# B-R-P/NMSLIB-ZIG

Measured on AMD Instinct MI355X. Metric: queries/sec @ recall@10, 1M x 128-D L2, batch=1024; HBM GB/s vs peak, higher is better.
Workload: dtype f16+f32

## Files before the change

nmslib_zig_amd/csrc/kernels/bf_kernels.hip:

```cpp
#include <cstdio>
#include <type_traits>
#include <vector>
#include <cstdlib>

#include "common_dev.hpp"
#include "kernels.hpp"

namespace gfxknn {

enum BfMode : int { BF_L2 = 0, BF_DOT = 1, BF_COS = 2, BF_L1 = 3, BF_LINF = 4, BF_COSC = 5, BF_L2D = 6 };

struct BfArgs {
    const float* base;
    const float* aux;
    const float* qaux;
    int aux_stride;
    const float* queries;
    u64* cand;
    int* cand_cnt;
    uint32_t* gthr;
    uint32_t* gq;
    int xj, xm;
    int n, ldb, nqt, nsplit, rows_per_split, kprime, cap;
    int kcs;
// ... 1422 lines not shown
                    if (have_pv) {
                        const float m = block_max(QG - 1, pv_ax);
                        mfma3_over(0, 0, true);
                        __builtin_amdgcn_sched_barrier(0);
                        finish_check(m, acc[QG - 1], QG - 1, pv_ax, pv_row0);
                    } else {
                        mfma3(0, 0, true, iv);
                    }
                    __builtin_amdgcn_sched_barrier(0);
#pragma unroll
                    for (int g = 1; g < QG; ++g) mfma3(g, 0, true, iv);
                } else if (kc == 7) {
                    mfma3(0, 7, false, acc[0]);
#pragma unroll
                    for (int g = 1; g < QG; ++g) {
                        __builtin_amdgcn_sched_barrier(0);
                        const float m = block_max(g - 1, axs + blk * 32);
                        mfma3_over(g, 7, false);
                        __builtin_amdgcn_sched_barrier(0);
                        finish_check(m, acc[g - 1], g - 1, axs + blk * 32, row0 + blk * 32);
                        __builtin_amdgcn_sched_barrier(0);
                    }
                } else {
#pragma unroll
                    for (int g = 0; g < QG; ++g) mfma3(g, kc, false, acc[0]);
                }
                __builtin_amdgcn_sched_barrier(0);
            }
            pv_ax = axs + blk * 32;
            pv_row0 = row0 + blk * 32;
            have_pv = true;
            if (blk == 0) {
                if (t + 2 < nstages) asm volatile("s_waitcnt vmcnt(9)\n\ts_barrier" ::: "memory");
                else asm volatile("s_waitcnt vmcnt(0)\n\ts_barrier" ::: "memory");
                if (t + kRing - 1 < nstages) issue_tile(t + kRing - 1);
            }
        }
    }
    asm volatile("s_waitcnt lgkmcnt(0)" ::: "memory");
    if (have_pv) finish_check(block_max(QG - 1, pv_ax), acc[QG - 1], QG - 1, pv_ax, pv_row0);
#pragma unroll
    for (int g = 0; g < QG; ++g) {
        const int qidx = (qt * NW + wave) * (32 * QG) + g * 32 + l31;
        if constexpr (SAMPLE) {
            float* o = a.top8 + (((size_t)qidx * a.nsplit + split) * 2 + h) * 8;
#pragma unroll
            for (int i = 0; i < 8; ++i) o[i] = t8[g][i];
        } else {
            a.list_cnt[((size_t)qidx * a.nsplit + split) * 2 + h] = cnt[g];
        }
    }
}

template <int MODE, bool SAMPLE, int QG, int NW, int KCH = 1>
__global__ __launch_bounds__(NW * 64) void bf_scan_bf16_kernel(BfScanF32Args a) {
    extern __shared__ __attribute__((aligned(16))) char smem[];
    const int tid = threadIdx.x, lane = tid & 63, wave = tid >> 6;
    const int h = lane >> 5, l31 = lane & 31;
    const int b = blockIdx.x;
    const int xcd = b & 7, rest = b >> 3;
    const int qt = rest % a.nqt;
    const int split = (rest / a.nqt) * 8 + xcd;
    if (split >= a.nsplit) return;
    if (a.group_flag && (a.group_flag[qt] != 0) != (a.group_want != 0)) return;

    constexpr int kSync = 4, kRing = 2 * kSync + 1, kAuxRing = 16, kStageBytes = BF_BN * 256;
    char* ring = smem;
    float* auxr = reinterpret_cast<float*>(ring + kRing * kStageBytes);
    const int tstr = SAMPLE ? a.tile_stride : 1;
    const int tiles_all = (a.n + BF_BN - 1) / BF_BN;
    const int stiles_all = (tiles_all + tstr - 1) / tstr;
    const int ntiles = max(0, min(a.tps, stiles_all - split * a.tps));
    const int nstages = ntiles * KCH;
    constexpr int kDp = 128 * KCH;
    const int r_begin = split * a.tps * tstr * BF_BN;
    const int stage_rows = tstr * BF_BN;

    uint32_t dma_voff[16 / NW];
#pragma unroll
    for (int jj = 0; jj < 16 / NW; ++jj) {
        const int pj = (16 / NW) * wave + jj;
        const int row = 4 * pj + (lane >> 4);
        const int c = (lane & 15) ^ (row & 15);
        dma_voff[jj] = (uint32_t)((row * kDp + c * 8) * 2);
    }
    const uint32_t dma_lds0 = (uint32_t)(uintptr_t)(lptr_t)ring + (uint32_t)((16 / NW) * __builtin_amdgcn_readfirstlane(wave) * 1024);
    const uint32_t aux_lds0 = (uint32_t)(uintptr_t)(lptr_t)auxr;
    const uint32_t aux_voff = (uint32_t)lane * 4u;
    auto issue_tile = [&](int stage) __attribute__((always_inline)) {
        const int slot = stage % kRing;
        const int row0 = r_begin + (stage / KCH) * stage_rows;
        const unsigned long long sbase = (unsigned long long)(uintptr_t)a.base_h16 + ((unsigned long long)row0 * kDp + (stage % KCH) * 128) * 2ull;
        const uint32_t m0v = dma_lds0 + (uint32_t)slot * kStageBytes;
#pragma clang diagnostic push
#pragma clang diagnostic ignored "-Winline-asm"
#pragma unroll
        for (int jj = 0; jj < 16 / NW; ++jj)
            asm volatile("s_mov_b32 m0, %2\n\ts_nop 0\n\tglobal_load_lds_dwordx4 %0, %1"
                         :: "v"(dma_voff[jj]), "s"(sbase), "s"(m0v + (uint32_t)jj * 1024u) : "memory", "m0");
        const unsigned long long abase = (unsigned long long)(uintptr_t)a.auxp16 + (unsigned long long)row0 * 4ull;
        asm volatile("s_mov_b32 m0, %2\n\ts_nop 0\n\tglobal_load_lds_dword %0, %1"
                     :: "v"(aux_voff), "s"(abase), "s"(aux_lds0 + (uint32_t)((stage % kAuxRing) * BF_BN * 4)) : "memory", "m0");
#pragma clang diagnostic pop
    };

    f16x8 qh[QG][8 * KCH];
    float thr[QG];
    int cnt[QG], ecnt[QG];
    uint32_t* lp[QG];
    float t8[SAMPLE ? QG : 1][8];
#pragma unroll
    for (int g = 0; g < QG; ++g) {
        const int qidx = (qt * NW + wave) * (32 * QG) + g * 32 + l31;
#pragma unroll
        for (int kc = 0; kc < 8 * KCH; ++kc)
            asm volatile("global_load_dwordx4 %0, %1, off" : "=a"(qh[g][kc]) : "v"(static_cast<const _Float16*>(a.q_h16) + (size_t)qidx * kDp + 16 * kc + 8 * h) : "memory");
        cnt[g] = 0;
        ecnt[g] = 0;
        if constexpr (SAMPLE) {
            thr[g] = -INFINITY;
            lp[g] = nullptr;
#pragma unroll
            for (int i = 0; i < 8; ++i) t8[g][i] = -INFINITY;
        } else {
            thr[g] = a.thr[qidx];
            lp[g] = a.list + (size_t)qidx * a.caph * (2 * a.nsplit) + split * 2 + h;
        }
    }
    asm volatile("s_waitcnt vmcnt(0)" ::: "memory");
    for (int t = 0; t <= kSync && t < nstages; ++t) issue_tile(t);
    asm volatile("s_waitcnt vmcnt(0)\n\ts_barrier" ::: "memory");

    uint32_t vad[8];
#pragma unroll
    for (int kc = 0; kc < 8; ++kc)
        vad[kc] = (uint32_t)(uintptr_t)(lptr_t)smem + (uint32_t)(l31 * 256 + (((kc * 2 + h) ^ (l31 & 15)) * 16));

    auto score_of = [&](const f32x16& c, int i, const float* ax) __attribute__((always_inline)) -> float {
        if constexpr (MODE == SC_COS) return c[i] * ax[(i & 3) + 8 * (i >> 2)];
        else return c[i];
    };
    auto block_max_leaves = [&](const f32x16& c, const float* ax, float (&m)[5]) __attribute__((always_inline)) {
#pragma unroll
        for (int j = 0; j < 5; ++j) {
            if constexpr (MODE == SC_COS)
                m[j] = fmaxf(fmaxf(score_of(c, 3 * j, ax), score_of(c, 3 * j + 1, ax)), score_of(c, 3 * j + 2, ax));
            else
                asm("v_max3_f32 %0, %1, %2, %3" : "=v"(m[j]) : "v"(c[3 * j]), "v"(c[3 * j + 1]), "v"(c[3 * j + 2]));
        }
    };
    auto block_max_root = [&](const f32x16& c, const float* ax, const float (&m)[5]) __attribute__((always_inline)) -> float {
        if constexpr (MODE == SC_COS) {
            return fmaxf(fmaxf(fmaxf(m[0], m[1]), m[2]), fmaxf(fmaxf(m[3], m[4]), score_of(c, 15, ax)));
        } else {
            float r0, r1, r;
            asm("v_max3_f32 %0, %1, %2, %3" : "=v"(r0) : "v"(m[0]), "v"(m[1]), "v"(m[2]));
            asm("v_max3_f32 %0, %1, %2, %3" : "=v"(r1) : "v"(m[3]), "v"(m[4]), "v"(c[15]));
            asm("v_max_f32 %0, %1, %2" : "=v"(r) : "v"(r0), "v"(r1));
            return r;
        }
    };
    auto block_max = [&](const f32x16& c, const float* ax) __attribute__((always_inline)) -> float {
        float m[5];
        block_max_leaves(c, ax, m);
        return block_max_root(c, ax, m);
    };
    auto trigger_of = [&](float m, int g) __attribute__((always_inline)) -> unsigned long long {
        return SAMPLE ? __builtin_amdgcn_ballot_w64(m > thr[g]) : __builtin_amdgcn_ballot_w64(m >= thr[g]);
    };
    auto finish_check = [&](unsigned long long trig, float m, const f32x16& c, int g, const float* ax, int row0) __attribute__((always_inline)) {
        if constexpr (SAMPLE) {
            if (__builtin_expect(trig != 0ull, 0)) {
                float v = (row0 + 32 <= a.n || MODE == SC_L2) ? m : -INFINITY;
#pragma unroll
                for (int j = 0; j < 8; ++j) {
                    const float hi = fmaxf(t8[g][j], v);
                    v = fminf(t8[g][j], v);
                    t8[g][j] = hi;
                }
                thr[g] = t8[g][7];
            }
        } else if (__builtin_expect(trig != 0ull, 0)) {
            uint32_t km;
            if constexpr (MODE == SC_COS) {
                f32x16 sc;
#pragma unroll
                for (int i = 0; i < 16; ++i) sc[i] = score_of(c, i, ax);
                km = hit_mask_f32(sc, thr[g]);
            } else {
                km = hit_mask_f32(c, thr[g]);
            }
            if (row0 + 32 > a.n) {
                int nvalid = a.n - row0;
                asm volatile("" : "+s"(nvalid));
#pragma unroll
                for (int i = 0; i < 16; ++i)
                    if (acc_row(i, h) >= nvalid) km &= ~(0x8000u >> i);
            }
            if (km) {
                if (ecnt[g] < a.caph) lp[g][(size_t)ecnt[g] * (2 * a.nsplit)] = ((uint32_t)(row0 - r_begin) >> 5 << 16) | km;
                ecnt[g]++;
                cnt[g] += __builtin_popcount(km);
            }
        }
    };

    f16x8 fh[4];
    f32x16 iv;
#pragma unroll
    for (int i = 0; i < 16; ++i) iv[i] = 0.f;
    f32x16 acc[2][QG];
#pragma unroll
    for (int g = 0; g < QG; ++g) {
#pragma unroll
        for (int i = 0; i < 16; ++i) {
            acc[0][g][i] = 0.f;
            acc[1][g][i] = -INFINITY;
        }
    }
    const float* pv_ax = auxr;
    int pv_row0 = 0;
    bool have_pv = false;
    float m_pend = 0.f;
    unsigned long long trig_pend = 0ull;
    const uint32_t lds0 = (uint32_t)(uintptr_t)(lptr_t)smem;
    auto load_frag = [&](auto off_tag, int kc) __attribute__((always_inline)) {
        constexpr int OFF = decltype(off_tag)::value;
        const uint32_t ad = vad[kc];
        if constexpr (NW == 4) {
            switch (kc % 4) {
                case 0: BF_FRAG_RD_OFF("v[224:227]", fh[0], ad, OFF); break;
                case 1: BF_FRAG_RD_OFF("v[228:231]", fh[1], ad, OFF); break;
                case 2: BF_FRAG_RD_OFF("v[232:235]", fh[2], ad, OFF); break;
                default: BF_FRAG_RD_OFF("v[236:239]", fh[3], ad, OFF); break;
            }
        } else {
            switch (kc % 4) {
                case 0: BF_FRAG_RD_OFF("v[96:99]", fh[0], ad, OFF); break;
                case 1: BF_FRAG_RD_OFF("v[100:103]", fh[1], ad, OFF); break;
                case 2: BF_FRAG_RD_OFF("v[104:107]", fh[2], ad, OFF); break;
                default: BF_FRAG_RD_OFF("v[108:111]", fh[3], ad, OFF); break;
            }
        }
    };
    using Off0 = std::integral_constant<int, 0>;
    using Off1 = std::integral_constant<int, 32 * 256>;
    auto wait_frag = [&](auto cnt_tag, int kc, bool with_init) __attribute__((always_inline)) {
        constexpr int N = decltype(cnt_tag)::value;
#define BF_W1(STR)                                                                                              \
        if constexpr (NW == 4) {                                                                                \
            switch (kc % 4) {                                                                                   \
                case 0:                                                                                         \
                    if (with_init) asm volatile(STR : "+{v[224:227]}"(fh[0]), "+{v[240:255]}"(iv));             \
                    else asm volatile(STR : "+{v[224:227]}"(fh[0]));                                            \
                    break;                                                                                      \
                case 1: asm volatile(STR : "+{v[228:231]}"(fh[1])); break;                                      \
                case 2: asm volatile(STR : "+{v[232:235]}"(fh[2])); break;                                      \
                default: asm volatile(STR : "+{v[236:239]}"(fh[3])); break;                                     \
            }                                                                                                   \
        } else {                                                                                                \
            switch (kc % 4) {                                                                                   \
                case 0:                                                                                         \
                    if (with_init) asm volatile(STR : "+{v[96:99]}"(fh[0]), "+{v[112:127]}"(iv));               \
                    else asm volatile(STR : "+{v[96:99]}"(fh[0]));                                              \
                    break;                                                                                      \
                case 1: asm volatile(STR : "+{v[100:103]}"(fh[1])); break;                                      \
                case 2: asm volatile(STR : "+{v[104:107]}"(fh[2])); break;                                      \
                default: asm volatile(STR : "+{v[108:111]}"(fh[3])); break;                                     \
            }                                                                                                   \
        }
        if constexpr (N == 0) { BF_W1("s_waitcnt lgkmcnt(0)") }
        else if constexpr (N == 2) { BF_W1("s_waitcnt lgkmcnt(2)") }
        else if constexpr (N == 3) { BF_W1("s_waitcnt lgkmcnt(3)") }
        else if constexpr (N == 6) { BF_W1("s_waitcnt lgkmcnt(6)") }
        else { static_assert(N == 7, "wait count"); BF_W1("s_waitcnt lgkmcnt(7)") }
#undef BF_W1
    };
    auto mfma_step = [&](f32x16& c, const f16x8& q, int kc, bool first_ch) __attribute__((always_inline)) {
        if constexpr (MODE == SC_L2) {
            if (kc == 0 && first_ch) {
                if constexpr (NW == 4)
                    asm("v_mfma_f32_32x32x16_f16 %0, %1, %2, %3" : "=&v"(c) : "{v[224:227]}"(fh[0]), "a"(q), "{v[240:255]}"(iv));
                else
                    asm("v_mfma_f32_32x32x16_f16 %0, %1, %2, %3" : "=&v"(c) : "{v[96:99]}"(fh[0]), "a"(q), "{v[112:127]}"(iv));
                return;
            }
        }
        c = __builtin_amdgcn_mfma_f32_32x32x16_f16(fh[kc % 4], q, (kc == 0 && first_ch) ? iv : c, 0, 0, 0);
    };
    auto load_init = [&](uint32_t ax) __attribute__((always_inline)) {
        if constexpr (MODE == SC_L2) {
            if constexpr (NW == 4)
                asm volatile("ds_read_b128 v[240:243], %1\n\tds_read_b128 v[244:247], %1 offset:32\n\t"
                             "ds_read_b128 v[248:251], %1 offset:64\n\tds_read_b128 v[252:255], %1 offset:96"
                             : "={v[240:255]}"(iv) : "v"(ax) : "memory");
            else
                asm volatile("ds_read_b128 v[112:115], %1\n\tds_read_b128 v[116:119], %1 offset:32\n\t"
                             "ds_read_b128 v[120:123], %1 offset:64\n\tds_read_b128 v[124:127], %1 offset:96"
                             : "={v[112:127]}"(iv) : "v"(ax) : "memory");
        }
    };
    constexpr int kInitReads = MODE == SC_L2 ? 4 : 0;
    const uint32_t aux_a = lds0 + kRing * kStageBytes + 16 * h;
    constexpr int kPre = 3;
    auto main_loop = [&](auto stag_tag) __attribute__((always_inline)) {
    constexpr int kStag = decltype(stag_tag)::value;
    if (kStag != 0 && a.prio_half) __builtin_amdgcn_s_setprio(1);
    load_init(aux_a);
#pragma unroll
    for (int kc = 0; kc < kPre; ++kc) load_frag(Off0{}, kc);
    for (int tt = 0; tt < ntiles; ++tt) {
#pragma unroll
      for (int ch = 0; ch < KCH; ++ch) {
        const int t = tt * KCH + ch;
        constexpr bool kOne = KCH == 1;
        const bool first_ch = kOne || ch == 0, last_ch = kOne || ch == KCH - 1;
        const float* axs = auxr + (t % kAuxRing) * BF_BN + 4 * h;
        const int row0 = r_begin + tt * stage_rows;
#pragma unroll
        for (int blk = 0; blk < 2; ++blk) {
            const bool prev_final = blk == 1 ? last_ch : first_ch;
            const bool init_next = blk == 0 ? first_ch : last_ch;
            const int dslot = ((t + 1) % kRing == 0) ? -(kRing - 1) * kStageBytes : kStageBytes;
            const uint32_t nax = blk == 0 ? aux_a + ((t % kAuxRing) * BF_BN + 32) * 4 : aux_a + (((t + 1) % kAuxRing) * BF_BN) * 4;
#pragma unroll
            for (int kc = 0; kc < 8; ++kc) {
                if (kc + kPre < 8) {
                    if (blk == 0) load_frag(Off0{}, kc + kPre);
                    else load_frag(Off1{}, kc + kPre);
                    wait_frag(std::integral_constant<int, kPre>{}, kc, kc == 0 && MODE == SC_L2 && first_ch);
                } else {
                    if (kc == 6 && init_next) load_init(nax);
                    if (blk == 0) {
                        load_frag(Off1{}, kc + kPre - 8);
                    } else {
                        vad[kc + kPre - 8] += (uint32_t)dslot;
                        load_frag(Off0{}, kc + kPre - 8);
                    }
                    if (kInitReads && init_next && kc >= 6) wait_frag(std::integral_constant<int, kPre + 4>{}, kc, false);
                    else wait_frag(std::integral_constant<int, kPre>{}, kc, false);
                }
                __builtin_amdgcn_sched_barrier(0);
                constexpr int kEvery = 8 / QG;
                const int gc = kc >= kStag ? (kc - kStag) / kEvery : 0;
                const bool chk = prev_final && kc >= kStag && ((kc - kStag) % kEvery) == 0;
                const bool br = prev_final && kc >= kStag && ((kc - kStag) % kEvery) == 1;
                float m = 0.f;
                const bool by_hand = MODE == SC_L2 && kc == 0 && first_ch && chk && QG == 2;
                float m5[5];
                if (chk && !by_hand) m = block_max(acc[blk ^ 1][gc], pv_ax);
                mfma_step(acc[blk][0], qh[0][8 * ch + kc], kc, first_ch);
                if (by_hand) {
                    if constexpr (QG == 2) {
                        __builtin_amdgcn_sched_barrier(0);
                        block_max_leaves(acc[blk ^ 1][gc], pv_ax, m5);
                        __builtin_amdgcn_sched_barrier(0);
                        mfma_step(acc[blk][1], qh[1][8 * ch + kc], kc, first_ch);
                        __builtin_amdgcn_sched_barrier(0);
                        m = block_max_root(acc[blk ^ 1][gc], pv_ax, m5);
                    }
                } else if (br) {
                    __builtin_amdgcn_sched_barrier(0);
                    finish_check(trig_pend, m_pend, acc[blk ^ 1][gc], gc, pv_ax, pv_row0);
                    __builtin_amdgcn_sched_barrier(0);
                } else {
                    __builtin_amdgcn_sched_group_barrier(0x008, 1, 0);
                    __builtin_amdgcn_sched_group_barrier(0x002, 12 / QG, 0);
                }
#pragma unroll
                for (int g = 1; g < QG; ++g) {
                    if (by_hand) break;
                    mfma_step(acc[blk][g], qh[g][8 * ch + kc], kc, first_ch);
                    __builtin_amdgcn_sched_group_barrier(0x008, 1, 0);
                    __builtin_amdgcn_sched_group_barrier(0x002, 12 / QG, 0);
                }
                if (chk) {
                    asm volatile("" : "+v"(m));
                    unsigned long long trig = trigger_of(m, gc);
                    asm volatile("" : "+s"(trig));
                    m_pend = m;
                    trig_pend = trig;
                }
                __builtin_amdgcn_sched_barrier(0);
            }
            if (last_ch) {
                pv_ax = axs + blk * 32;
                pv_row0 = row0 + blk * 32;
                have_pv = true;
            }
            if (blk == 1) {
#pragma unroll
                for (int kc = kPre; kc < 8; ++kc) vad[kc] += (uint32_t)dslot;
            }
            if (blk == 0) {
                if (t % kSync == 0) {
                    asm volatile("s_waitcnt vmcnt(0)\n\ts_barrier" ::: "memory");
                    for (int u = t + kSync + 1; u <= t + 2 * kSync && u < nstages; ++u) issue_tile(u);
                }
            }
        }
      }
    }
    asm volatile("s_waitcnt lgkmcnt(0)" ::: "memory");
    };
    if constexpr (NW == 8) {
        if (__builtin_amdgcn_readfirstlane(wave) >= 4) main_loop(std::integral_constant<int, 2>{});
        else main_loop(std::integral_constant<int, 0>{});
    } else {
        main_loop(std::integral_constant<int, 0>{});
    }
    if (have_pv) {
#pragma unroll
        for (int g = 0; g < QG; ++g) {
            const float m = block_max(acc[1][g], pv_ax);
            finish_check(trigger_of(m, g), m, acc[1][g], g, pv_ax, pv_row0);
        }
    }
#pragma unroll
    for (int g = 0; g < QG; ++g) {
        const int qidx = (qt * NW + wave) * (32 * QG) + g * 32 + l31;
        if constexpr (SAMPLE) {
            float* o = a.top8 + (((size_t)qidx * a.nsplit + split) * 2 + h) * 8;
#pragma unroll
            for (int i = 0; i < 8; ++i) o[i] = t8[g][i];
        } else {
            a.list_cnt[((size_t)qidx * a.nsplit + split) * 2 + h] = cnt[g];
        }
    }
}

__global__ void split_bf16_kernel(const float* src, int rows, int rows_pad, int ld, int dim, __bf16* hi, __bf16* lo,
                                  const float* aux, float aux_pad, float* auxp, int dp, _Float16* h16, float scale,
                                  float* auxp16, float aux16_mul) {
    const size_t total = (size_t)rows_pad * dp;
    for (size_t i = (size_t)blockIdx.x * blockDim.x + threadIdx.x; i < total; i += (size_t)gridDim.x * blockDim.x) {
        const size_t r = i / (size_t)dp;
        const int c = (int)(i - r * dp);
        const float v = (r < (size_t)rows && c < dim) ? src[r * ld + c] : 0.f;
        const __bf16 hh = (__bf16)v;
        if (hi) hi[i] = hh;
        if (lo) lo[i] = (__bf16)(v - (float)hh);
        if (h16) h16[i] = (_Float16)(scale * v);
        if (c == 0 && auxp) auxp[r] = r < (size_t)rows ? (aux ? aux[r] : 0.f) : aux_pad;
        if (c == 0 && auxp16) auxp16[r] = r < (size_t)rows ? (aux ? aux[r] * aux16_mul : 0.f) : aux_pad;
    }
}

__global__ void bf_f32_prep_kernel(const float* raw, int nq, int dim, const float* sel, int qpad, int ld, float* pad_out,
                                   __bf16* hi, __bf16* lo, int* clr0, int n0, int* clr1, int n1, uint32_t* clr2, size_t n2,
                                   int dp, _Float16* h16, float scale) {
    const size_t gtid = (size_t)blockIdx.x * blockDim.x + threadIdx.x, gsz = (size_t)gridDim.x * blockDim.x;
    const size_t total = (size_t)qpad * dp;
    for (size_t i = gtid; i < total; i += gsz) {
        const size_t r = i / (size_t)dp;
        const int c = (int)(i - r * dp);
        float v;
        if (raw) {
            v = (r < (size_t)nq && c < dim) ? raw[r * dim + c] : 0.f;
            if (c < ld) pad_out[r * ld + c] = v;
        } else {
            v = c < dim ? sel[r * ld + c] : 0.f;
        }
        const __bf16 hh = (__bf16)v;
        if (hi) hi[i] = hh;
        if (lo) lo[i] = (__bf16)(v - (float)hh);
        h16[i] = (_Float16)(scale * v);
    }
    for (size_t i = gtid; i < (size_t)n0; i += gsz) clr0[i] = 0;
// ... 135 lines not shown
        int run = incl - sum;
        for (int i = 0; i < per; ++i) {
            const int s = tid * per + i;
            if (s < nl) {
                offs[s] = run;
                const int c = a.list_cnt[(size_t)q * nl + s];
                run += c < a.caph ? c : a.caph;
            }
        }
        if (tid == 63) offs[nl] = incl;
        if (__any(over != 0) && tid == 0) s_over = 1;
    } else if (wave == 1) {
        const bool split_product = a.precise[q / a.fail_queries] != 0;
        const float* qs = a.queries_sel + (size_t)q * a.sel_ld;
        float ss = 0.f;
        for (int d = lane; d < a.sel_dim; d += 64) ss = fmaf(qs[d], qs[d], ss);
        ss = wave_sum(ss);
        const float e1 = split_product ? 0.f : one_product_error(qs, a.sel_dim, lane, a.scale * (a.space == SP_L2 || a.space == SP_NEGDOT || a.qaux ? a.bmax : 1.0f), a.bres16, a.scale_q);
        if (lane == 0) {
            s_qn2 = ss;
            s_e1 = e1;
            s_split = split_product ? 1 : 0;
            s_thr = split_product ? a.thr[q] : a.thr1[q];
        }
    }
    __syncthreads();
    const int total = offs[nl];
    if ((a.no_split && a.precise[q / a.fail_queries] != 0) ||
        (a.qaux && a.qaux[(size_t)q * 4 + 3] == 0.f)) {
        if (tid == 0) atomicOr(&a.tile_fail[q / a.fail_queries], 1);
        return;
    }
    const int need = a.k < a.n ? a.k : a.n;
    const int want = need + (a.k / 8 > 4 ? a.k / 8 : 4) < a.n ? need + (a.k / 8 > 4 ? a.k / 8 : 4) : a.n;
    if (s_over || total < want || total > a.p2max) {
        if (tid == 0) atomicOr(&a.tile_fail[q / a.fail_queries], 1);
        return;
    }
    lap(0);
    scan_gather_entries(keys, offs, a.list, q, nl, a.caph, a.tps, tid, blockDim.x);
    __syncthreads();
    lap(1);
    const int P = next_pow2(total < 2 ? 2 : total);
    if (a.prof && tid == 0) {
        atomicAdd(&a.prof[8], (unsigned long long)total);
        atomicAdd(&a.prof[9], (unsigned long long)P);
        atomicAdd(&a.prof[10], 1ull);
    }
    const float* qq = a.queries + (size_t)q * a.ldb;
    const int sub = lane & 15, rg = lane >> 4;
    if (a.dim <= 128) {
        float qv[8];
        bool ok[8];
    #pragma unroll
        for (int c = 0; c < 8; ++c) {
            const int d = sub + 16 * c;
            ok[c] = d < a.dim;
            qv[c] = ok[c] ? qq[d] : 0.f;
        }
        constexpr int kU = 4;
        for (int j0 = wave * (4 * kU); j0 < total; j0 += 16 * kU) {
            uint32_t pos[kU];
            float xv[kU][8];
    #pragma unroll
            for (int u = 0; u < kU; ++u) {
                const int j = j0 + 4 * u + rg;
                pos[u] = (uint32_t)keys[j < total ? j : total - 1];
                const float* row = a.base + (size_t)pos[u] * a.ldb + sub;
    #pragma unroll
                for (int c = 0; c < 8; ++c) xv[u][c] = ok[c] ? row[16 * c] : 0.f;
            }
            __builtin_amdgcn_wave_barrier();
    #pragma unroll
            for (int u = 0; u < kU; ++u) {
                float p0[4], p1[4], p2[4];
    #pragma unroll
                for (int v = 0; v < 4; ++v) {
                    p0[v] = p1[v] = p2[v] = 0.f;
    #pragma unroll
                    for (int c = 0; c < 2; ++c) {
                        if (64 * c >= a.dim) continue;
                        const float x = xv[u][v + 4 * c], y = qv[v + 4 * c];
                        if (a.space == SP_L2) {
                            const float t = x - y;
                            p0[v] = fmaf(t, t, p0[v]);
                        } else {
                            p0[v] = fmaf(x, y, p0[v]);
                            if (a.space != SP_NEGDOT) {
                                p1[v] = fmaf(x, x, p1[v]);
                                p2[v] = fmaf(y, y, p2[v]);
                            }
                        }
                    }
                }
                auto tree = [&](const float* p) __attribute__((always_inline)) -> float {
                    float s = (p[0] + p[2]) + (p[1] + p[3]);
    #pragma unroll
                    for (int o = 8; o > 0; o >>= 1) s += __shfl_xor(s, o, 64);
                    return s;
                };
                const float s0 = tree(p0);
                float d;
                if (a.space == SP_L2) d = sqrtf(s0);
                else if (a.space == SP_NEGDOT) d = -s0;
                else {
                    const float sim = normdot_finish(s0, tree(p1), tree(p2));
                    d = a.space == SP_ANGULAR ? acosf(sim) : fmaxf(0.0f, 1.0f - sim);
                }
                const int j = j0 + 4 * u + rg;
                if (sub == 0 && j < total) keys[j] = ((u64)f32_ord(d) << 32) | pos[u];
            }
        }
    } else {
        const int nstep = (a.dim + 63) >> 6;
        for (int j0 = wave * 16; j0 < total; j0 += 64) {
            uint32_t pos[4];
            const float* rowp[4];
    #pragma unroll
            for (int u = 0; u < 4; ++u) {
                const int j = j0 + 4 * u + rg;
                pos[u] = (uint32_t)keys[j < total ? j : total - 1];
                rowp[u] = a.base + (size_t)pos[u] * a.ldb + sub;
            }
            float p0[4][4], p1[4][4], p2[4][4];
    #pragma unroll
            for (int u = 0; u < 4; ++u)
    #pragma unroll
                for (int v = 0; v < 4; ++v) p0[u][v] = p1[u][v] = p2[u][v] = 0.f;
            for (int c0 = 0; c0 < nstep; c0 += 2) {
                float xv[4][8], qv[8];
                bool ok[8];
    #pragma unroll
                for (int c = 0; c < 8; ++c) {
                    const int d = sub + 16 * (c & 3) + 64 * (c0 + (c >> 2));
                    ok[c] = d < a.dim;
                    qv[c] = ok[c] ? qq[d] : 0.f;
    #pragma unroll
                    for (int u = 0; u < 4; ++u) xv[u][c] = ok[c] ? rowp[u][16 * (c & 3) + 64 * (c0 + (c >> 2))] : 0.f;
                }
    #pragma unroll
                for (int u = 0; u < 4; ++u) {
    #pragma unroll
                    for (int v = 0; v < 4; ++v) {
    #pragma unroll
                        for (int c = 0; c < 2; ++c) {
                            if (64 * (c0 + c) >= a.dim) continue;
                            const float x = xv[u][v + 4 * c], y = qv[v + 4 * c];
                            if (a.space == SP_L2) {
                                const float t = x - y;
                                p0[u][v] = fmaf(t, t, p0[u][v]);
                            } else {
                                p0[u][v] = fmaf(x, y, p0[u][v]);
                                if (a.space != SP_NEGDOT) {
                                    p1[u][v] = fmaf(x, x, p1[u][v]);
                                    p2[u][v] = fmaf(y, y, p2[u][v]);
                                }
                            }
                        }
                    }
                }
            }
            __builtin_amdgcn_wave_barrier();
    #pragma unroll
            for (int u = 0; u < 4; ++u) {
                auto tree = [&](const float* p) __attribute__((always_inline)) -> float {
                    float s = (p[0] + p[2]) + (p[1] + p[3]);
    #pragma unroll
                    for (int o = 8; o > 0; o >>= 1) s += __shfl_xor(s, o, 64);
                    return s;
                };
                const float s0 = tree(p0[u]);
                float d;
                if (a.space == SP_L2) d = sqrtf(s0);
                else if (a.space == SP_NEGDOT) d = -s0;
                else {
                    const float sim = normdot_finish(s0, tree(p1[u]), tree(p2[u]));
                    d = a.space == SP_ANGULAR ? acosf(sim) : fmaxf(0.0f, 1.0f - sim);
                }
                const int j = j0 + 4 * u + rg;
                if (sub == 0 && j < total) keys[j] = ((u64)f32_ord(d) << 32) | pos[u];
            }
        }
    }
    __syncthreads();
    lap(2);
    if (total <= 512 && a.k <= 32) {
        __shared__ u64 s_head[128];
        const int e0 = wave * 128 + 2 * lane;
        u64 k0 = e0 < total ? keys[e0] : ~0ull, k1 = e0 + 1 < total ? keys[e0 + 1] : ~0ull;
        wave_sort128_u64(k0, k1, lane);
        if (lane < 16) {
            s_head[wave * 32 + 2 * lane] = k0;
            s_head[wave * 32 + 2 * lane + 1] = k1;
        }
        __syncthreads();
        if (wave == 0) {
            k0 = s_head[2 * lane];
            k1 = s_head[2 * lane + 1];
            wave_sort128_u64(k0, k1, lane);
            if (lane < 16) {
                keys[2 * lane] = k0;
                keys[2 * lane + 1] = k1;
            }
        }
        __syncthreads();
    } else {
        for (int i = total + tid; i < P; i += blockDim.x) keys[i] = ~0ull;
        __syncthreads();
        block_bitonic_u64_asc(keys, P, tid, blockDim.x);
    }
    lap(3);
    const int found = total < a.k ? total : a.k;
    if (total < a.n) {
        const bool split_product = s_split != 0;
        if (tid == 0) {
            const float qn2 = s_qn2, qn = sqrtf(qn2);
            const float dk = ord_f32((uint32_t)(keys[found - 1] >> 32));
            float sk, e, extra = 0.f;
            if (a.qaux) {
                const float sh = sinf(0.5f * dk);
// ... 1005 lines not shown
    f.caph = caph;
    f.p2max = host_next_pow2((int)(2.5 * f.rcap * f.stride) + 64);
    if (f.p2max > 2 * ns * caph) f.p2max = host_next_pow2(2 * ns * caph);
    f.lds_scan = 4 * 2 * BF_BN * 256 + 8 * BF_BN * 4 + 64;
    f.lds_scan1 = 9 * BF_BN * 256 + 16 * BF_BN * 4 + 64;
    f.lds_rerank = (size_t)f.p2max * 8 + (2 * (size_t)ns + 1) * 4 + 16;
    const int stiles = (tiles_all + f.stride - 1) / f.stride;
    const int s_nqt = f.qpad / (f.kch > 1 ? 128 : 256);
    int nss = (256 + s_nqt - 1) / s_nqt;
    if (nss > stiles / 16) nss = stiles / 16;
    if (nss > 64) nss = 64;
    nss = (nss + 7) / 8 * 8;
    if (nss < 8) nss = 8;
    f.s_nsplit = nss;
    f.s_tps = (stiles + nss - 1) / nss;
    f.lds_thr = (size_t)host_next_pow2(nss * 2 * 8) * 8 + 16;
    f.fallback = bf_make_plan(n, dim_rows, nq, k, false, tq);
    if (f.kch > 1) f.force_precise = false;
    return f;
}

hipError_t launch_row_maxnorm(const float* rows, int n, int ld, int dim, bool relative_residual, float* out, hipStream_t s,
                              float scale16) {
    hipError_t e = hipMemsetAsync(out, 0, 16, s);
    if (e != hipSuccess || n == 0) return e;
    int grid = (n + 3) / 4;
    if (grid > 4096) grid = 4096;
    hipLaunchKernelGGL(row_maxnorm_kernel, dim3(grid), dim3(256), 0, s, rows, n, ld, dim, relative_residual ? 1 : 0,
                       reinterpret_cast<unsigned*>(out), scale16);
    return hipGetLastError();
}

hipError_t launch_split_bf16(const float* src, int rows, int rows_pad, int ld, int dim, void* hi, void* lo,
                             const float* aux, float aux_pad, float* auxp, hipStream_t s, int dp, void* h16, float scale,
                             float* auxp16, float aux16_mul) {
    const size_t total = (size_t)rows_pad * dp;
    if (total == 0) return hipSuccess;
    size_t grid = (total + 255) / 256;
    if (grid > 16384) grid = 16384;
    hipLaunchKernelGGL(split_bf16_kernel, dim3((unsigned)grid), dim3(256), 0, s, src, rows, rows_pad, ld, dim,
                       static_cast<__bf16*>(hi), static_cast<__bf16*>(lo), aux, aux_pad, auxp, dp, static_cast<_Float16*>(h16),
                       scale, auxp16, aux16_mul);
    return hipGetLastError();
}

template <int MODE, bool SAMPLE, int QG>
static hipError_t launch_scan_f32_one(const BfScanF32Args& a, int grid, size_t lds, hipStream_t s) {
    hipError_t e = hipFuncSetAttribute(reinterpret_cast<const void*>(bf_scan_f32_kernel<MODE, SAMPLE, QG>),
                                       hipFuncAttributeMaxDynamicSharedMemorySize, (int)lds);
    if (e != hipSuccess) return e;
    hipLaunchKernelGGL((bf_scan_f32_kernel<MODE, SAMPLE, QG>), dim3(grid), dim3(256), lds, s, a);
    return hipGetLastError();
}
template <int MODE, bool SAMPLE, int QG, int NW>
static hipError_t launch_scan_bf16_one(const BfScanF32Args& a, int grid, size_t lds, hipStream_t s) {
    hipError_t e = hipFuncSetAttribute(reinterpret_cast<const void*>(bf_scan_bf16_kernel<MODE, SAMPLE, QG, NW>),
                                       hipFuncAttributeMaxDynamicSharedMemorySize, (int)lds);
    if (e != hipSuccess) return e;
    hipLaunchKernelGGL((bf_scan_bf16_kernel<MODE, SAMPLE, QG, NW>), dim3(grid), dim3(NW * 64), lds, s, a);
    return hipGetLastError();
}
template <int MODE>
static hipError_t launch_scan_f32_mode(const BfScanF32Args& a, bool sample, int terms, int qg, int grid, size_t lds, hipStream_t s, int kch = 1) {
    if (kch > 1) {
        if (terms != 1) return hipSuccess;
        auto go = [&](auto kern) -> hipError_t {
            hipError_t e = hipFuncSetAttribute(reinterpret_cast<const void*>(kern), hipFuncAttributeMaxDynamicSharedMemorySize, (int)lds);
            if (e != hipSuccess) return e;
            hipLaunchKernelGGL(kern, dim3(grid), dim3(256), lds, s, a);
            return hipGetLastError();
        };
        switch (kch) {
            case 2: return sample ? go(bf_scan_bf16_kernel<MODE, true, 1, 4, 2>) : go(bf_scan_bf16_kernel<MODE, false, 1, 4, 2>);
            case 3: return sample ? go(bf_scan_bf16_kernel<MODE, true, 1, 4, 3>) : go(bf_scan_bf16_kernel<MODE, false, 1, 4, 3>);
            case 4: return sample ? go(bf_scan_bf16_kernel<MODE, true, 1, 4, 4>) : go(bf_scan_bf16_kernel<MODE, false, 1, 4, 4>);
            case 6: return sample ? go(bf_scan_bf16_kernel<MODE, true, 1, 4, 6>) : go(bf_scan_bf16_kernel<MODE, false, 1, 4, 6>);
            case 8: return sample ? go(bf_scan_bf16_kernel<MODE, true, 1, 4, 8>) : go(bf_scan_bf16_kernel<MODE, false, 1, 4, 8>);
            default: return hipErrorInvalidValue;
        }
    }
    const char* w8e = getenv("NMSLIB_GPU_BF16_W8");
    const int w8 = w8e ? atoi(w8e) : 7;
    if (sample) return (w8 & 4) ? launch_scan_bf16_one<MODE, true, 1, 8>(a, grid, lds, s) : launch_scan_bf16_one<MODE, true, 2, 4>(a, grid, lds, s);
    if (terms == 1) {
        if (qg == 2) return (w8 & 1) ? launch_scan_bf16_one<MODE, false, 2, 8>(a, grid, lds, s) : launch_scan_bf16_one<MODE, false, 4, 4>(a, grid, lds, s);
        return (w8 & 2) ? launch_scan_bf16_one<MODE, false, 1, 8>(a, grid, lds, s) : launch_scan_bf16_one<MODE, false, 2, 4>(a, grid, lds, s);
    }
    if (qg == 2) return launch_scan_f32_one<MODE, false, 4>(a, grid, lds, s);
    return launch_scan_f32_one<MODE, false, 2>(a, grid, lds, s);
}

hipError_t launch_bf_f32_fast(const BfF32Fast& f, int space, int n, int dim, int ldb, int nq, int k, const float* base_orig,
                              const float* sel_rows, const float* aux, const void* base_hi, const void* base_lo,
                              const float* auxp, float bmax, float bres, const float* queries_orig, const float* queries_sel,
                              void* q_hi, void* q_lo, float* top8, unsigned long long* cand_fb, int* cnt_fb, float* thr,
                              uint32_t* list, int* list_cnt, int* tile_fail, int* flags_fb, const int32_t* ext_ids,
                              int32_t* out_ids, float* out_dists, int32_t* out_cnt, hipEvent_t scan_begin,
                              hipEvent_t scan_end, hipStream_t s, const float* queries_raw, float* queries_pad_out,
                              const float* qaux_cosc, const float* queries_centred, int sel_ld, const BfF16Side& h16) {
    const int sdim = f.cosc ? f.sel_dim : dim, sld = f.cosc ? sel_ld : ldb;
    float* thr1 = thr + f.qpad;
    int* precise = tile_fail + f.nqt;
    hipError_t e;
    {
        const BfPlan& fb = f.fallback;
        uint32_t* gthr = reinterpret_cast<uint32_t*>(cnt_fb + (size_t)fb.qpad * fb.nsplit);
        const size_t gwords = 2 * ((size_t)fb.qpad + (size_t)fb.qpad * fb.nsplit);
        size_t work = (size_t)f.qpad * f.dp > gwords ? (size_t)f.qpad * f.dp : gwords;
        size_t grid = (work + 255) / 256;
        if (grid > 2048) grid = 2048;
        hipLaunchKernelGGL(bf_f32_prep_kernel, dim3((unsigned)grid), dim3(256), 0, s, queries_raw, nq, sdim, queries_sel, f.qpad,
                           sld, queries_pad_out, f.kch > 1 ? nullptr : static_cast<__bf16*>(q_hi),
                           f.kch > 1 ? nullptr : static_cast<__bf16*>(q_lo),
                           tile_fail, 2 * f.nqt, flags_fb, fb.nqt, gthr, gwords, f.dp, static_cast<_Float16*>(h16.q_h16), h16.scale_q);
        e = hipGetLastError();
        if (e != hipSuccess) return e;
    }
    auto scan = [&](const BfScanF32Args& sa, bool sample, int terms, int grid) -> hipError_t {
        const size_t lds = terms == 1 ? f.lds_scan1 : f.lds_scan;
        if (f.mode == 0) return launch_scan_f32_mode<SC_L2>(sa, sample, terms, f.qg, grid, lds, s, f.kch);
        if (f.mode == 1) return launch_scan_f32_mode<SC_DOT>(sa, sample, terms, f.qg, grid, lds, s, f.kch);
        return launch_scan_f32_mode<SC_COS>(sa, sample, terms, f.qg, grid, lds, s, f.kch);
    };
    BfScanF32Args a{};
    a.base_hi = static_cast<const __bf16*>(base_hi);
    a.base_lo = static_cast<const __bf16*>(base_lo);
    a.auxp = auxp;
    a.q_hi = static_cast<const __bf16*>(q_hi);
    a.q_lo = static_cast<const __bf16*>(q_lo);
    a.base_h16 = h16.base_h16;
    {
        static const int prio = getenv("NMSLIB_GPU_BF16_PRIO") ? atoi(getenv("NMSLIB_GPU_BF16_PRIO")) : 0;
        a.prio_half = prio;
    }
    a.q_h16 = h16.q_h16;
    a.auxp16 = h16.auxp16;
    a.n = n;
    a.nqt = f.nqt;
    BfScanF32Args sa = a;
// ... 233 lines not shown
```

Baseline: 2.872 million.

## Use 16x16x32 MFMA shape for eight-wave bf16 scan kernel

Adds an S16 variant of the half-precision scan kernel that computes each 32-row tile with four 16x16x32 MFMAs instead of one 32x32x16. Query fragment loads, LDS fragment addressing, the L2 bias init and the block-max reduction (using permlane16 swaps) are adapted to the new accumulator layout. The new variant becomes the default for the eight-wave launches, with an env var to fall back to the 32x32 shape. It is meant to shorten MFMA dependency latency and interleave the max reduction better, at the cost of more instructions and extra lane shuffles on the hit path.

```diff
diff --git a/nmslib_zig_amd/csrc/kernels/bf_kernels.hip b/nmslib_zig_amd/csrc/kernels/bf_kernels.hip
--- a/nmslib_zig_amd/csrc/kernels/bf_kernels.hip
+++ b/nmslib_zig_amd/csrc/kernels/bf_kernels.hip
@@ -1498,11 +1498,13 @@
     }
 }
 
-template <int MODE, bool SAMPLE, int QG, int NW, int KCH = 1>
+template <int MODE, bool SAMPLE, int QG, int NW, int KCH = 1, bool S16 = false>
 __global__ __launch_bounds__(NW * 64) void bf_scan_bf16_kernel(BfScanF32Args a) {
+    static_assert(!S16 || (NW == 8 && KCH == 1), "the 16x16 shape serves the eight-wave, one-chunk scan");
     extern __shared__ __attribute__((aligned(16))) char smem[];
     const int tid = threadIdx.x, lane = tid & 63, wave = tid >> 6;
     const int h = lane >> 5, l31 = lane & 31;
+    const int l15 = lane & 15, e16 = (lane >> 4) & 1;
     const int b = blockIdx.x;
     const int xcd = b & 7, rest = b >> 3;
     const int qt = rest % a.nqt;
@@ -1559,8 +1561,14 @@
     for (int g = 0; g < QG; ++g) {
         const int qidx = (qt * NW + wave) * (32 * QG) + g * 32 + l31;
 #pragma unroll
-        for (int kc = 0; kc < 8 * KCH; ++kc)
-            asm volatile("global_load_dwordx4 %0, %1, off" : "=a"(qh[g][kc]) : "v"(static_cast<const _Float16*>(a.q_h16) + (size_t)qidx * kDp + 16 * kc + 8 * h) : "memory");
+        for (int kc = 0; kc < 8 * KCH; ++kc) {
+            if constexpr (S16) {
+                const int qb = qidx - l31 + 16 * (kc & 1) + l15;
+                asm volatile("global_load_dwordx4 %0, %1, off" : "=a"(qh[g][kc]) : "v"(static_cast<const _Float16*>(a.q_h16) + (size_t)qb * kDp + 32 * (kc >> 1) + 8 * (lane >> 4)) : "memory");
+            } else {
+                asm volatile("global_load_dwordx4 %0, %1, off" : "=a"(qh[g][kc]) : "v"(static_cast<const _Float16*>(a.q_h16) + (size_t)qidx * kDp + 16 * kc + 8 * h) : "memory");
+            }
+        }
         cnt[g] = 0;
         ecnt[g] = 0;
         if constexpr (SAMPLE) {
@@ -1579,8 +1587,14 @@
 
     uint32_t vad[8];
 #pragma unroll
-    for (int kc = 0; kc < 8; ++kc)
-        vad[kc] = (uint32_t)(uintptr_t)(lptr_t)smem + (uint32_t)(l31 * 256 + (((kc * 2 + h) ^ (l31 & 15)) * 16));
+    for (int kc = 0; kc < 8; ++kc) {
+        if constexpr (S16) {
+            const int row = (l15 & 3) + 8 * (2 * (kc & 1) + ((l15 >> 2) & 1)) + 4 * (l15 >> 3);
+            vad[kc] = (uint32_t)(uintptr_t)(lptr_t)smem + (uint32_t)(row * 256 + (((4 * (kc >> 1) + (lane >> 4)) ^ (row & 15)) * 16));
+        } else {
+            vad[kc] = (uint32_t)(uintptr_t)(lptr_t)smem + (uint32_t)(l31 * 256 + (((kc * 2 + h) ^ (l31 & 15)) * 16));
+        }
+    }
 
     auto score_of = [&](const f32x16& c, int i, const float* ax) __attribute__((always_inline)) -> float {
         if constexpr (MODE == SC_COS) return c[i] * ax[(i & 3) + 8 * (i >> 2)];
@@ -1650,18 +1664,64 @@
             }
         }
     };
+    auto half_max16 = [&](const f32x4& lo, const f32x4& hi, const float* ax) __attribute__((always_inline)) -> float {
+        if constexpr (MODE == SC_COS) {
+            const float* x = ax + 8 * e16;
+            return fmaxf(fmaxf(fmaxf(lo[0] * x[0], lo[1] * x[1]), fmaxf(lo[2] * x[2], lo[3] * x[3])),
+                         fmaxf(fmaxf(hi[0] * x[16], hi[1] * x[17]), fmaxf(hi[2] * x[18], hi[3] * x[19])));
+        } else {
+            float p0, p1, r;
+            asm("v_max3_f32 %0, %1, %2, %3" : "=v"(p0) : "v"(lo[0]), "v"(lo[1]), "v"(lo[2]));
+            asm("v_max3_f32 %0, %1, %2, %3" : "=v"(p1) : "v"(lo[3]), "v"(hi[0]), "v"(hi[1]));
+            asm("v_max3_f32 %0, %1, %2, %3" : "=v"(p0) : "v"(p0), "v"(p1), "v"(hi[2]));
+            asm("v_max_f32 %0, %1, %2" : "=v"(r) : "v"(p0), "v"(hi[3]));
+            return r;
+        }
+    };
+    auto swap_max16 = [&](float ma, float mb) __attribute__((always_inline)) -> float {
+        float r;
+        asm("s_nop 1\n\tv_permlane16_swap_b32 %0, %1" : "+v"(ma), "+v"(mb));
+        asm("v_max_f32 %0, %1, %2" : "=v"(r) : "v"(ma), "v"(mb));
+        return r;
+    };
+    auto block_max16 = [&](const f32x4 (&c)[4], const float* ax) __attribute__((always_inline)) -> float {
+        return swap_max16(half_max16(c[0], c[2], ax), half_max16(c[1], c[3], ax));
+    };
+    auto finish_check16 = [&](unsigned long long trig, float m, const f32x4 (&c)[4], int g, const float* ax, int row0) __attribute__((always_inline)) {
+        if constexpr (SAMPLE) {
+            f32x16 none = {};
+            finish_check(trig, m, none, g, ax, row0);
+        } else if (__builtin_expect(trig != 0ull, 0)) {
+            f32x16 o;
+#pragma unroll
+            for (int rt = 0; rt < 2; ++rt) {
+#pragma unroll
+                for (int i = 0; i < 4; ++i) {
+                    float x = c[2 * rt][i], y = c[2 * rt + 1][i];
+                    asm volatile("s_nop 1\n\tv_permlane16_swap_b32 %0, %1" : "+v"(x), "+v"(y));
+                    o[i + 8 * rt] = x;
+                    o[i + 8 * rt + 4] = y;
+                }
+            }
+            finish_check(trig, m, o, g, ax, row0);
+        }
+    };
 
     f16x8 fh[4];
     f32x16 iv;
 #pragma unroll
     for (int i = 0; i < 16; ++i) iv[i] = 0.f;
     f32x16 acc[2][QG];
+    f32x4 acc4[2][QG][4];
+    f32x4 iv0, iv1;
 #pragma unroll
     for (int g = 0; g < QG; ++g) {
 #pragma unroll
         for (int i = 0; i < 16; ++i) {
             acc[0][g][i] = 0.f;
             acc[1][g][i] = -INFINITY;
+            acc4[0][g][i >> 2][i & 3] = 0.f;
+            acc4[1][g][i >> 2][i & 3] = -INFINITY;
         }
     }
     const float* pv_ax = auxr;
@@ -1707,7 +1767,9 @@
         } else {                                                                                                \
             switch (kc % 4) {                                                                                   \
                 case 0:                                                                                         \
-                    if (with_init) asm volatile(STR : "+{v[96:99]}"(fh[0]), "+{v[112:127]}"(iv));               \
+                    if (with_init && S16)                                                                       \
+                        asm volatile(STR : "+{v[96:99]}"(fh[0]), "+{v[112:115]}"(iv0), "+{v[116:119]}"(iv1));   \
+                    else if (with_init) asm volatile(STR : "+{v[96:99]}"(fh[0]), "+{v[112:127]}"(iv));          \
                     else asm volatile(STR : "+{v[96:99]}"(fh[0]));                                              \
                     break;                                                                                      \
                 case 1: asm volatile(STR : "+{v[100:103]}"(fh[1])); break;                                      \
@@ -1718,6 +1780,7 @@
         if constexpr (N == 0) { BF_W1("s_waitcnt lgkmcnt(0)") }
         else if constexpr (N == 2) { BF_W1("s_waitcnt lgkmcnt(2)") }
         else if constexpr (N == 3) { BF_W1("s_waitcnt lgkmcnt(3)") }
+        else if constexpr (N == 5) { BF_W1("s_waitcnt lgkmcnt(5)") }
         else if constexpr (N == 6) { BF_W1("s_waitcnt lgkmcnt(6)") }
         else { static_assert(N == 7, "wait count"); BF_W1("s_waitcnt lgkmcnt(7)") }
 #undef BF_W1
@@ -1734,8 +1797,23 @@
         }
         c = __builtin_amdgcn_mfma_f32_32x32x16_f16(fh[kc % 4], q, (kc == 0 && first_ch) ? iv : c, 0, 0, 0);
     };
+    auto mfma16 = [&](f32x4& c, const f16x8& q, int kc) __attribute__((always_inline)) {
+        if (kc < 2) {
+            if constexpr (MODE == SC_L2) {
+                if (kc == 0) asm("v_mfma_f32_16x16x32_f16 %0, %1, %2, %3" : "=&v"(c) : "{v[96:99]}"(fh[0]), "a"(q), "{v[112:115]}"(iv0));
+                else asm("v_mfma_f32_16x16x32_f16 %0, %1, %2, %3" : "=&v"(c) : "{v[100:103]}"(fh[1]), "a"(q), "{v[116:119]}"(iv1));
+            } else {
+                c = __builtin_amdgcn_mfma_f32_16x16x32_f16(fh[kc % 4], q, f32x4{0.f, 0.f, 0.f, 0.f}, 0, 0, 0);
+            }
+            return;
+        }
+        c = __builtin_amdgcn_mfma_f32_16x16x32_f16(fh[kc % 4], q, c, 0, 0, 0);
+    };
     auto load_init = [&](uint32_t ax) __attribute__((always_inline)) {
-        if constexpr (MODE == SC_L2) {
+        if constexpr (MODE == SC_L2 && S16) {
+            asm volatile("ds_read_b128 v[112:115], %2\n\tds_read_b128 v[116:119], %2 offset:64"
+                         : "={v[112:115]}"(iv0), "={v[116:119]}"(iv1) : "v"(ax) : "memory");
+        } else if constexpr (MODE == SC_L2) {
             if constexpr (NW == 4)
                 asm volatile("ds_read_b128 v[240:243], %1\n\tds_read_b128 v[244:247], %1 offset:32\n\t"
                              "ds_read_b128 v[248:251], %1 offset:64\n\tds_read_b128 v[252:255], %1 offset:96"
@@ -1746,8 +1824,8 @@
                              : "={v[112:127]}"(iv) : "v"(ax) : "memory");
         }
     };
-    constexpr int kInitReads = MODE == SC_L2 ? 4 : 0;
-    const uint32_t aux_a = lds0 + kRing * kStageBytes + 16 * h;
+    constexpr int kInitReads = MODE == SC_L2 ? (S16 ? 2 : 4) : 0;
+    const uint32_t aux_a = lds0 + kRing * kStageBytes + 16 * h + (S16 ? 32 * e16 : 0);
     constexpr int kPre = 3;
     auto main_loop = [&](auto stag_tag) __attribute__((always_inline)) {
     constexpr int kStag = decltype(stag_tag)::value;
@@ -1783,7 +1861,7 @@
                         vad[kc + kPre - 8] += (uint32_t)dslot;
                         load_frag(Off0{}, kc + kPre - 8);
                     }
-                    if (kInitReads && init_next && kc >= 6) wait_frag(std::integral_constant<int, kPre + 4>{}, kc, false);
+                    if (kInitReads && init_next && kc >= 6) wait_frag(std::integral_constant<int, kPre + kInitReads>{}, kc, false);
                     else wait_frag(std::integral_constant<int, kPre>{}, kc, false);
                 }
                 __builtin_amdgcn_sched_barrier(0);
@@ -1792,33 +1870,79 @@
                 const bool chk = prev_final && kc >= kStag && ((kc - kStag) % kEvery) == 0;
                 const bool br = prev_final && kc >= kStag && ((kc - kStag) % kEvery) == 1;
                 float m = 0.f;
-                const bool by_hand = MODE == SC_L2 && kc == 0 && first_ch && chk && QG == 2;
-                float m5[5];
-                if (chk && !by_hand) m = block_max(acc[blk ^ 1][gc], pv_ax);
-                mfma_step(acc[blk][0], qh[0][8 * ch + kc], kc, first_ch);
-                if (by_hand) {
-                    if constexpr (QG == 2) {
+                if constexpr (S16) {
+                    const int rt = kc & 1, kk = kc >> 1;
+                    const bool by_hand16 = MODE == SC_L2 && kc == 0 && chk && QG == 2;
+                    if (by_hand16) {
+                        if constexpr (QG == 2) {
+                            float ma, mb;
+                            mfma16(acc4[blk][0][2 * rt], qh[0][2 * kk], kc);
+                            __builtin_amdgcn_sched_barrier(0);
+                            ma = half_max16(acc4[blk ^ 1][gc][0], acc4[blk ^ 1][gc][2], pv_ax);
+                            __builtin_amdgcn_sched_barrier(0);
+                            mfma16(acc4[blk][0][2 * rt + 1], qh[0][2 * kk + 1], kc);
+                            __builtin_amdgcn_sched_barrier(0);
+                            mb = half_max16(acc4[blk ^ 1][gc][1], acc4[blk ^ 1][gc][3], pv_ax);
+                            __builtin_amdgcn_sched_barrier(0);
+                            mfma16(acc4[blk][1][2 * rt], qh[1][2 * kk], kc);
+                            __builtin_amdgcn_sched_barrier(0);
+                            m = swap_max16(ma, mb);
+                            __builtin_amdgcn_sched_barrier(0);
+                            mfma16(acc4[blk][1][2 * rt + 1], qh[1][2 * kk + 1], kc);
+                        }
+                    } else {
+                        if (chk) m = block_max16(acc4[blk ^ 1][gc], pv_ax);
+                        mfma16(acc4[blk][0][2 * rt], qh[0][2 * kk], kc);
+                        if (br) {
+                            __builtin_amdgcn_sched_barrier(0);
+                            finish_check16(trig_pend, m_pend, acc4[blk ^ 1][gc], gc, pv_ax, pv_row0);
+                            __builtin_amdgcn_sched_barrier(0);
+                        } else {
+                            __builtin_amdgcn_sched_group_barrier(0x008, 1, 0);
+                            __builtin_amdgcn_sched_group_barrier(0x002, 6 / QG, 0);
+                        }
+                        mfma16(acc4[blk][0][2 * rt + 1], qh[0][2 * kk + 1], kc);
+                        __builtin_amdgcn_sched_group_barrier(0x008, 1, 0);
+                        __builtin_amdgcn_sched_group_barrier(0x002, 6 / QG, 0);
+#pragma unroll
+                        for (int g = 1; g < QG; ++g) {
+#pragma unroll
+                            for (int qt = 0; qt < 2; ++qt) {
+                                mfma16(acc4[blk][g][2 * rt + qt], qh[g][2 * kk + qt], kc);
+                                __builtin_amdgcn_sched_group_barrier(0x008, 1, 0);
+                                __builtin_amdgcn_sched_group_barrier(0x002, 6 / QG, 0);
+                            }
+                        }
+                    }
+                } else {
+                    const bool by_hand = MODE == SC_L2 && kc == 0 && first_ch && chk && QG == 2;
+                    float m5[5];
+                    if (chk && !by_hand) m = block_max(acc[blk ^ 1][gc], pv_ax);
+                    mfma_step(acc[blk][0], qh[0][8 * ch + kc], kc, first_ch);
+                    if (by_hand) {
+                        if constexpr (QG == 2) {
+                            __builtin_amdgcn_sched_barrier(0);
+                            block_max_leaves(acc[blk ^ 1][gc], pv_ax, m5);
+                            __builtin_amdgcn_sched_barrier(0);
+                            mfma_step(acc[blk][1], qh[1][8 * ch + kc], kc, first_ch);
+                            __builtin_amdgcn_sched_barrier(0);
+                            m = block_max_root(acc[blk ^ 1][gc], pv_ax, m5);
+                        }
+                    } else if (br) {
                         __builtin_amdgcn_sched_barrier(0);
-                        block_max_leaves(acc[blk ^ 1][gc], pv_ax, m5);
+                        finish_check(trig_pend, m_pend, acc[blk ^ 1][gc], gc, pv_ax, pv_row0);
                         __builtin_amdgcn_sched_barrier(0);
-                        mfma_step(acc[blk][1], qh[1][8 * ch + kc], kc, first_ch);
-                        __builtin_amdgcn_sched_barrier(0);
-                        m = block_max_root(acc[blk ^ 1][gc], pv_ax, m5);
+                    } else {
+                        __builtin_amdgcn_sched_group_barrier(0x008, 1, 0);
+                        __builtin_amdgcn_sched_group_barrier(0x002, 12 / QG, 0);
                     }
-                } else if (br) {
-                    __builtin_amdgcn_sched_barrier(0);
-                    finish_check(trig_pend, m_pend, acc[blk ^ 1][gc], gc, pv_ax, pv_row0);
-                    __builtin_amdgcn_sched_barrier(0);
-                } else {
-                    __builtin_amdgcn_sched_group_barrier(0x008, 1, 0);
-                    __builtin_amdgcn_sched_group_barrier(0x002, 12 / QG, 0);
-                }
-#pragma unroll
-                for (int g = 1; g < QG; ++g) {
-                    if (by_hand) break;
-                    mfma_step(acc[blk][g], qh[g][8 * ch + kc], kc, first_ch);
-                    __builtin_amdgcn_sched_group_barrier(0x008, 1, 0);
-                    __builtin_amdgcn_sched_group_barrier(0x002, 12 / QG, 0);
+#pragma unroll
+                    for (int g = 1; g < QG; ++g) {
+                        if (by_hand) break;
+                        mfma_step(acc[blk][g], qh[g][8 * ch + kc], kc, first_ch);
+                        __builtin_amdgcn_sched_group_barrier(0x008, 1, 0);
+                        __builtin_amdgcn_sched_group_barrier(0x002, 12 / QG, 0);
+                    }
                 }
                 if (chk) {
                     asm volatile("" : "+v"(m));
@@ -1858,8 +1982,13 @@
     if (have_pv) {
 #pragma unroll
         for (int g = 0; g < QG; ++g) {
-            const float m = block_max(acc[1][g], pv_ax);
-            finish_check(trigger_of(m, g), m, acc[1][g], g, pv_ax, pv_row0);
+            if constexpr (S16) {
+                const float m = block_max16(acc4[1][g], pv_ax);
+                finish_check16(trigger_of(m, g), m, acc4[1][g], g, pv_ax, pv_row0);
+            } else {
+                const float m = block_max(acc[1][g], pv_ax);
+                finish_check(trigger_of(m, g), m, acc[1][g], g, pv_ax, pv_row0);
+            }
         }
     }
 #pragma unroll
@@ -2101,7 +2230,7 @@
     if (a.dim <= 128) {
         float qv[8];
         bool ok[8];
-    #pragma unroll
+#pragma unroll
         for (int c = 0; c < 8; ++c) {
             const int d = sub + 16 * c;
             ok[c] = d < a.dim;
@@ -2111,22 +2240,22 @@
         for (int j0 = wave * (4 * kU); j0 < total; j0 += 16 * kU) {
             uint32_t pos[kU];
             float xv[kU][8];
-    #pragma unroll
+#pragma unroll
             for (int u = 0; u < kU; ++u) {
                 const int j = j0 + 4 * u + rg;
                 pos[u] = (uint32_t)keys[j < total ? j : total - 1];
                 const float* row = a.base + (size_t)pos[u] * a.ldb + sub;
-    #pragma unroll
+#pragma unroll
                 for (int c = 0; c < 8; ++c) xv[u][c] = ok[c] ? row[16 * c] : 0.f;
             }
             __builtin_amdgcn_wave_barrier();
-    #pragma unroll
+#pragma unroll
             for (int u = 0; u < kU; ++u) {
                 float p0[4], p1[4], p2[4];
-    #pragma unroll
+#pragma unroll
                 for (int v = 0; v < 4; ++v) {
                     p0[v] = p1[v] = p2[v] = 0.f;
-    #pragma unroll
+#pragma unroll
                     for (int c = 0; c < 2; ++c) {
                         if (64 * c >= a.dim) continue;
                         const float x = xv[u][v + 4 * c], y = qv[v + 4 * c];
@@ -2144,7 +2273,7 @@
                 }
                 auto tree = [&](const float* p) __attribute__((always_inline)) -> float {
                     float s = (p[0] + p[2]) + (p[1] + p[3]);
-    #pragma unroll
+#pragma unroll
                     for (int o = 8; o > 0; o >>= 1) s += __shfl_xor(s, o, 64);
                     return s;
                 };
@@ -2165,33 +2294,33 @@
         for (int j0 = wave * 16; j0 < total; j0 += 64) {
             uint32_t pos[4];
             const float* rowp[4];
-    #pragma unroll
+#pragma unroll
             for (int u = 0; u < 4; ++u) {
                 const int j = j0 + 4 * u + rg;
                 pos[u] = (uint32_t)keys[j < total ? j : total - 1];
                 rowp[u] = a.base + (size_t)pos[u] * a.ldb + sub;
             }
             float p0[4][4], p1[4][4], p2[4][4];
-    #pragma unroll
+#pragma unroll
             for (int u = 0; u < 4; ++u)
-    #pragma unroll
+#pragma unroll
                 for (int v = 0; v < 4; ++v) p0[u][v] = p1[u][v] = p2[u][v] = 0.f;
             for (int c0 = 0; c0 < nstep; c0 += 2) {
                 float xv[4][8], qv[8];
                 bool ok[8];
-    #pragma unroll
+#pragma unroll
                 for (int c = 0; c < 8; ++c) {
                     const int d = sub + 16 * (c & 3) + 64 * (c0 + (c >> 2));
                     ok[c] = d < a.dim;
                     qv[c] = ok[c] ? qq[d] : 0.f;
-    #pragma unroll
+#pragma unroll
                     for (int u = 0; u < 4; ++u) xv[u][c] = ok[c] ? rowp[u][16 * (c & 3) + 64 * (c0 + (c >> 2))] : 0.f;
                 }
-    #pragma unroll
+#pragma unroll
                 for (int u = 0; u < 4; ++u) {
-    #pragma unroll
+#pragma unroll
                     for (int v = 0; v < 4; ++v) {
-    #pragma unroll
+#pragma unroll
                         for (int c = 0; c < 2; ++c) {
                             if (64 * (c0 + c) >= a.dim) continue;
                             const float x = xv[u][v + 4 * c], y = qv[v + 4 * c];
@@ -2210,11 +2339,11 @@
                 }
             }
             __builtin_amdgcn_wave_barrier();
-    #pragma unroll
+#pragma unroll
             for (int u = 0; u < 4; ++u) {
                 auto tree = [&](const float* p) __attribute__((always_inline)) -> float {
                     float s = (p[0] + p[2]) + (p[1] + p[3]);
-    #pragma unroll
+#pragma unroll
                     for (int o = 8; o > 0; o >>= 1) s += __shfl_xor(s, o, 64);
                     return s;
                 };
@@ -3326,13 +3455,19 @@
     hipLaunchKernelGGL((bf_scan_f32_kernel<MODE, SAMPLE, QG>), dim3(grid), dim3(256), lds, s, a);
     return hipGetLastError();
 }
-template <int MODE, bool SAMPLE, int QG, int NW>
+template <int MODE, bool SAMPLE, int QG, int NW, bool S16 = false>
 static hipError_t launch_scan_bf16_one(const BfScanF32Args& a, int grid, size_t lds, hipStream_t s) {
-    hipError_t e = hipFuncSetAttribute(reinterpret_cast<const void*>(bf_scan_bf16_kernel<MODE, SAMPLE, QG, NW>),
+    hipError_t e = hipFuncSetAttribute(reinterpret_cast<const void*>(bf_scan_bf16_kernel<MODE, SAMPLE, QG, NW, 1, S16>),
                                        hipFuncAttributeMaxDynamicSharedMemorySize, (int)lds);
     if (e != hipSuccess) return e;
-    hipLaunchKernelGGL((bf_scan_bf16_kernel<MODE, SAMPLE, QG, NW>), dim3(grid), dim3(NW * 64), lds, s, a);
+    hipLaunchKernelGGL((bf_scan_bf16_kernel<MODE, SAMPLE, QG, NW, 1, S16>), dim3(grid), dim3(NW * 64), lds, s, a);
     return hipGetLastError();
+}
+template <int MODE, bool SAMPLE, int QG>
+static hipError_t launch_scan_bf16_w8(const BfScanF32Args& a, int grid, size_t lds, hipStream_t s) {
+    const char* se = getenv("NMSLIB_GPU_BF16_SHAPE");
+    if (se && atoi(se) == 32) return launch_scan_bf16_one<MODE, SAMPLE, QG, 8>(a, grid, lds, s);
+    return launch_scan_bf16_one<MODE, SAMPLE, QG, 8, true>(a, grid, lds, s);
 }
 template <int MODE>
 static hipError_t launch_scan_f32_mode(const BfScanF32Args& a, bool sample, int terms, int qg, int grid, size_t lds, hipStream_t s, int kch = 1) {
@@ -3355,10 +3490,10 @@
     }
     const char* w8e = getenv("NMSLIB_GPU_BF16_W8");
     const int w8 = w8e ? atoi(w8e) : 7;
-    if (sample) return (w8 & 4) ? launch_scan_bf16_one<MODE, true, 1, 8>(a, grid, lds, s) : launch_scan_bf16_one<MODE, true, 2, 4>(a, grid, lds, s);
+    if (sample) return (w8 & 4) ? launch_scan_bf16_w8<MODE, true, 1>(a, grid, lds, s) : launch_scan_bf16_one<MODE, true, 2, 4>(a, grid, lds, s);
     if (terms == 1) {
-        if (qg == 2) return (w8 & 1) ? launch_scan_bf16_one<MODE, false, 2, 8>(a, grid, lds, s) : launch_scan_bf16_one<MODE, false, 4, 4>(a, grid, lds, s);
-        return (w8 & 2) ? launch_scan_bf16_one<MODE, false, 1, 8>(a, grid, lds, s) : launch_scan_bf16_one<MODE, false, 2, 4>(a, grid, lds, s);
+        if (qg == 2) return (w8 & 1) ? launch_scan_bf16_w8<MODE, false, 2>(a, grid, lds, s) : launch_scan_bf16_one<MODE, false, 4, 4>(a, grid, lds, s);
+        return (w8 & 2) ? launch_scan_bf16_w8<MODE, false, 1>(a, grid, lds, s) : launch_scan_bf16_one<MODE, false, 2, 4>(a, grid, lds, s);
     }
     if (qg == 2) return launch_scan_f32_one<MODE, false, 4>(a, grid, lds, s);
     return launch_scan_f32_one<MODE, false, 2>(a, grid, lds, s);
```

Measured after the change: 2.926 million, median of 6. No clear change (+1.9%).
